# BloodAxe/pytorch-toolbelt

Measured on AMD Instinct MI355X. Metric: megapixels/sec tiled+d4-TTA merge on 5000x5000, higher is better.
Workload: dtype f32

## Files before the change

### pytorch_toolbelt_amd/csrc/ptb_bandplan.hip

```cpp
#include <algorithm>
#include <vector>

#include "ptb_view_device.h"

namespace ptb {

constexpr int PLAN_TILES = 224;
constexpr int PLAN_CH = 32;

struct BandItem {
    int ax, ay;
    int cwch;
    int ntiles;
    int partial;
    int pad[3];
    unsigned long long cover[MAX_COVER];
};
static_assert(sizeof(BandItem) == 64, "BandItem layout");

struct GroupTiles {
    const void* src[PLAN_TILES];
    long long vs[PLAN_TILES];
};

template <int NV, int CODES, int OPK, int LD, int CH = PLAN_CH, bool PF = false>
__global__ __launch_bounds__(16 * CH) void band_plan_kernel(const ViewArgs a, const BandItem* __restrict__ items, const GroupTiles t) {
    constexpr bool DB = PF && CH == 64 && lds_tiles(NV, CODES) > 0;
    constexpr int LDS_SET = lds_tiles(NV, CODES) * CW * CH;
    __shared__ __attribute__((aligned(16))) float lds[LDS_SET ? LDS_SET * (DB ? 2 : 1) : 4];
    const int tid = threadIdx.x;
    unsigned bid = blockIdx.x;
    if (a.ncells == 1) {
        const unsigned per_xcd = ((unsigned)a.total_chunks + 7u) / 8u;
        bid = (blockIdx.x & 7u) * per_xcd + (blockIdx.x >> 3);
        if (bid >= (unsigned)a.total_chunks) return;
    }
    int c = bid % a.C;
    unsigned item = bid / a.C;
    if (a.chan_loop) { c = 0; item = bid; }
    else if (a.ncells == 2) {
        const unsigned n_items = (unsigned)a.total_chunks / (unsigned)a.C;
        c = bid / n_items;
        item = bid - c * n_items;
    }
    const BandItem* __restrict__ it = items + item;
    const int cwch = it->cwch, partial = it->partial;
    const int cw = cwch & 0xffff, ch = cwch >> 16;
    const int q = tid & 15, r = tid >> 4;
    const bool act = (r < ch) && (4 * q < cw);
    const long long pix = (long long)(it->ay + r) * a.dst_row_stride + it->ax + 4 * q;
    float4 nfull = make_float4(1.f, 1.f, 1.f, 1.f);
    if (act && !partial) nfull = *reinterpret_cast<const float4*>(a.norm_full + pix);
    float4 acc = make_float4(0.f, 0.f, 0.f, 0.f);
    const int nt = it->ntiles;
    const bool rot = PF && a.rot_views && (item & 1u);
    constexpr bool ALL = PF && lds_tiles(NV, CODES) == 0 && NV <= 2 && CODES >= 0;
    if constexpr (ALL) {
        const int c_end = a.chan_loop ? a.C : c + 1;
        if (a.chan_loop) { c = 0; }
        float4 wv[MAX_COVER];
#pragma unroll
        for (int e = 0; e < MAX_COVER; ++e) {
            wv[e] = make_float4(0.f, 0.f, 0.f, 0.f);
            if (e < nt && act) {
                const unsigned long long cv = it->cover[e];
                const int lx = (int)((cv >> 16) & 0xffff), ly = (int)((cv >> 32) & 0xffff);
                wv[e] = *reinterpret_cast<const float4*>(a.weight + (long long)(ly + r) * a.W + lx + 4 * q);
            }
        }
        typename RawOf<LD>::type all[MAX_COVER][NV];
        auto request = [&](int cc) {
#pragma unroll
            for (int e = 0; e < MAX_COVER; ++e) {
                if (e < nt) {
                    const unsigned long long cv = it->cover[e];
                    const int slot = (int)(cv & 0xffff), lx = (int)((cv >> 16) & 0xffff), ly = (int)((cv >> 32) & 0xffff);
                    gather_load_raw<CH, NV, CODES, LD>(static_cast<const float*>(t.src[slot]), (long long)cc * a.H * a.W, t.vs[slot], a.nviews, a.codes, a.H,
                                                       a.W, lx, ly, cw, ch, tid, all[e]);
                }
            }
        };
        request(c);
        for (; c < c_end; ++c) {
            acc = make_float4(0.f, 0.f, 0.f, 0.f);
#pragma unroll
            for (int e = 0; e < MAX_COVER; ++e) {
                if (e < nt) {
                    float4 v[NV];
                    gather_widen<CH, NV, CODES, LD>(all[e], a.nviews, a.codes, cw, ch, tid, v);
                    float4 val = gather_tail<CH, NV, CODES, OPK>(v, a.nviews, a.codes, cw, ch, a.op, a.divisor, lds, tid, false);
                    val = round_src4<LD>(val, a.round_src);
                    acc.x = __fadd_rn(acc.x, __fmul_rn(val.x, wv[e].x));
                    acc.y = __fadd_rn(acc.y, __fmul_rn(val.y, wv[e].y));
                    acc.z = __fadd_rn(acc.z, __fmul_rn(val.z, wv[e].z));
                    acc.w = __fadd_rn(acc.w, __fmul_rn(val.w, wv[e].w));
                }
            }
            if (c + 1 < c_end) request(c + 1);
            if (act) {
                float* o = a.merged + (long long)c * a.dst_chan_stride + pix;
                if (partial) *reinterpret_cast<float4*>(o) = acc;
                else out_store4(o, make_float4(__fdiv_rn(acc.x, nfull.x), __fdiv_rn(acc.y, nfull.y), __fdiv_rn(acc.z, nfull.z), __fdiv_rn(acc.w, nfull.w)));
            }
        }
        return;
    }
    typename RawOf<LD>::type nxt[PF ? NV : 1];
    float4 wnxt = make_float4(0.f, 0.f, 0.f, 0.f);
    if constexpr (PF) {
        if (nt > 0) {
            const unsigned long long cv = it->cover[0];
            const int slot = (int)(cv & 0xffff), lx = (int)((cv >> 16) & 0xffff), ly = (int)((cv >> 32) & 0xffff);
            if (act) wnxt = *reinterpret_cast<const float4*>(a.weight + (long long)(ly + r) * a.W + lx + 4 * q);
            if (NV >= 2 && rot)
                gather_load_raw<CH, NV, CODES, LD, NV / 2>(static_cast<const float*>(t.src[slot]), (long long)c * a.H * a.W, t.vs[slot], a.nviews, a.codes, a.H,
                                                           a.W, lx, ly, cw, ch, tid, nxt);
            else
                gather_load_raw<CH, NV, CODES, LD>(static_cast<const float*>(t.src[slot]), (long long)c * a.H * a.W, t.vs[slot], a.nviews, a.codes, a.H, a.W, lx,
                                                   ly, cw, ch, tid, nxt);
        }
    }
    for (int e = 0; e < nt; ++e) {
        const unsigned long long cv = it->cover[e];
        const int slot = (int)(cv & 0xffff), lx = (int)((cv >> 16) & 0xffff), ly = (int)((cv >> 32) & 0xffff);
        float4 val;
        float4 w4 = make_float4(0.f, 0.f, 0.f, 0.f);
        if constexpr (PF) {
            float4 v[NV];
            gather_widen<CH, NV, CODES, LD>(nxt, a.nviews, a.codes, cw, ch, tid, v);
            w4 = wnxt;
            if (e + 1 < nt) {
                const unsigned long long cn = it->cover[e + 1];
                const int sn = (int)(cn & 0xffff), nlx = (int)((cn >> 16) & 0xffff), nly = (int)((cn >> 32) & 0xffff);
                if (act) wnxt = *reinterpret_cast<const float4*>(a.weight + (long long)(nly + r) * a.W + nlx + 4 * q);
                if (NV >= 2 && rot)
                    gather_load_raw<CH, NV, CODES, LD, NV / 2>(static_cast<const float*>(t.src[sn]), (long long)c * a.H * a.W, t.vs[sn], a.nviews, a.codes, a.H,
                                                               a.W, nlx, nly, cw, ch, tid, nxt);
                else
                    gather_load_raw<CH, NV, CODES, LD>(static_cast<const float*>(t.src[sn]), (long long)c * a.H * a.W, t.vs[sn], a.nviews, a.codes, a.H, a.W,
                                                       nlx, nly, cw, ch, tid, nxt);
            }
            const bool db = DB && a.lds_db;
            val = gather_tail<CH, NV, CODES, OPK>(v, a.nviews, a.codes, cw, ch, a.op, a.divisor, db ? lds + (e & 1) * LDS_SET : lds, tid, db ? false : e + 1 < nt);
        } else {
            val = gather_reduce<CH, NV, CODES, OPK, LD>(static_cast<const float*>(t.src[slot]), (long long)c * a.H * a.W, t.vs[slot],
                                                        a.nviews, a.codes, a.H, a.W, lx, ly, cw, ch, a.op, a.divisor, lds, tid,
                                                        e + 1 < nt);
            if (act) w4 = *reinterpret_cast<const float4*>(a.weight + (long long)(ly + r) * a.W + lx + 4 * q);
        }
        val = round_src4<LD>(val, a.round_src);
        if (act) {
            acc.x = __fadd_rn(acc.x, __fmul_rn(val.x, w4.x));
            acc.y = __fadd_rn(acc.y, __fmul_rn(val.y, w4.y));
            acc.z = __fadd_rn(acc.z, __fmul_rn(val.z, w4.z));
            acc.w = __fadd_rn(acc.w, __fmul_rn(val.w, w4.w));
        }
    }
    if (act) {
        float* o = a.merged + (long long)c * a.dst_chan_stride + pix;
        if (partial) *reinterpret_cast<float4*>(o) = acc;
        else out_store4(o, make_float4(__fdiv_rn(acc.x, nfull.x), __fdiv_rn(acc.y, nfull.y), __fdiv_rn(acc.z, nfull.z),
                                       __fdiv_rn(acc.w, nfull.w)));
    }
}

static void launch_plan(const ViewArgs& a, const BandItem* items, const GroupTiles& t, int blocks, int ch, hipStream_t s) {
    const dim3 grid(blocks), block(16 * ch);
    const bool nonlinear = a.op >= PTB_RED_GMEAN;
#define PTB_PLAN_PF(NV, CODES, LD)                                                                                  \
    do {                                                                                                            \
        if (ch == 64) {                                                                                             \
            if (nonlinear) hipLaunchKernelGGL((band_plan_kernel<NV, CODES, 1, LD, 64, true>), grid, block, 0, s, a, items, t); \
            else hipLaunchKernelGGL((band_plan_kernel<NV, CODES, 0, LD, 64, true>), grid, block, 0, s, a, items, t);       \
        } else if (nonlinear) hipLaunchKernelGGL((band_plan_kernel<NV, CODES, 1, LD, PLAN_CH, true>), grid, block, 0, s, a, items, t);    \
        else hipLaunchKernelGGL((band_plan_kernel<NV, CODES, 0, LD, PLAN_CH, true>), grid, block, 0, s, a, items, t);              \
    } while (0)
#define PTB_PLAN_LD(NV, CODES, LD)                                                                                  \
    do {                                                                                                            \
        if (ch == 64) {                                                                                             \
            if (nonlinear) hipLaunchKernelGGL((band_plan_kernel<NV, CODES, 1, LD, 64>), grid, block, 0, s, a, items, t); \
            else hipLaunchKernelGGL((band_plan_kernel<NV, CODES, 0, LD, 64>), grid, block, 0, s, a, items, t);       \
        } else if (nonlinear) hipLaunchKernelGGL((band_plan_kernel<NV, CODES, 1, LD>), grid, block, 0, s, a, items, t);    \
        else hipLaunchKernelGGL((band_plan_kernel<NV, CODES, 0, LD>), grid, block, 0, s, a, items, t);              \
    } while (0)
#define PTB_PLAN(NV, CODES)                                                                                         \
    do {                                                                                                            \
        if (a.in_dtype == PTB_F16) { if (g_band_half_pf) PTB_PLAN_PF(NV, CODES, 2); else PTB_PLAN_LD(NV, CODES, 2); }      \
        else if (a.in_dtype == PTB_BF16) { if (g_band_half_pf) PTB_PLAN_PF(NV, CODES, 3); else PTB_PLAN_LD(NV, CODES, 3); } \
        else if (g_band_half_pf >= 2) PTB_PLAN_PF(NV, CODES, 1);                                                    \
        else PTB_PLAN_LD(NV, CODES, 1);                                                                             \
    } while (0)
#define PTB_PLAN_RT(NV, CODES)           \
    do {                                                                                                            \
        if (a.in_dtype == PTB_F16) PTB_PLAN_LD(NV, CODES, 2);                                                       \
        else if (a.in_dtype == PTB_BF16) PTB_PLAN_LD(NV, CODES, 3);                                                 \
        else PTB_PLAN_LD(NV, CODES, 1);                                                                             \
    } while (0)
    if (a.nviews == 1 && a.codes == CODES_ID) PTB_PLAN(1, CODES_ID);
    else if (a.nviews == 2 && a.codes == CODES_FLIPLR) PTB_PLAN(2, CODES_FLIPLR);
    else if (a.nviews == 2 && a.codes == CODES_FLIPUD) PTB_PLAN(2, CODES_FLIPUD);
    else if (a.nviews == 3 && a.codes == CODES_FLIPS) PTB_PLAN(3, CODES_FLIPS);
    else if (a.nviews == 4 && a.codes == CODES_D2) PTB_PLAN(4, CODES_D2);
    else if (a.nviews == 8 && a.codes == CODES_D4) PTB_PLAN(8, CODES_D4);
    else PTB_PLAN_RT(8, -1);
#undef PTB_PLAN
#undef PTB_PLAN_RT
#undef PTB_PLAN_LD
#undef PTB_PLAN_PF
}

struct Group {
    int y0, y1;
    std::vector<int> tiles;
    int last_tile;
    long long item_off;
    int item_cnt;
};

}

struct ptb_band_plan {
    int n, C, th, tw, H, W;
    int ch = ptb::PLAN_CH;
    std::vector<int> xs, ys;
    std::vector<ptb::BandItem> items;
    std::vector<ptb::Group> groups;
    std::vector<int> last_group;
    std::vector<std::vector<int>> ready;
    std::vector<int> band_y0, band_y1, band_group;
    std::vector<char> group_launched;
    const ptb::BandItem* dev_items = nullptr;
    int n_bands = 0;
    int pos = 0, launched = 0;
    std::vector<const void*> src;
    std::vector<long long> vs;
    int cfg_set = 0, cfg_dtype = 0, cfg_V = 0, cfg_codes = 0, cfg_red = 0;
    int cfg_views[ptb::MAX_VIEWS] = {0};
    const void *cfg_merged = nullptr, *cfg_norm = nullptr, *cfg_weight = nullptr;
    struct Held { uintptr_t p0, p1; int last_group; };
    std::vector<Held> held;
    bool monotone = true;
};

using namespace ptb;

static int band_items(const ptb_band_plan& p, const std::vector<int>& cover, const std::vector<int>& slot_of, int y0, int y1, int partial,
                      std::vector<BandItem>& out) {
    std::vector<int> xe{0, p.W};
    for (int t : cover) { xe.push_back(p.xs[t]); xe.push_back(p.xs[t] + p.tw); }
    std::sort(xe.begin(), xe.end());
    xe.erase(std::unique(xe.begin(), xe.end()), xe.end());
    struct XCell { int ox, w, n; int tile[MAX_COVER]; };
    std::vector<XCell> cells;
    for (size_t xi = 0; xi + 1 < xe.size(); ++xi) {
        XCell c{};
        c.ox = xe[xi]; c.w = xe[xi + 1] - xe[xi];
        for (int t : cover) {
            if (p.xs[t] <= c.ox && c.ox < p.xs[t] + p.tw) {
                if (c.n == MAX_COVER) return PTB_EUNSUPPORTED;
                c.tile[c.n++] = t;
            }
        }
        if (!cells.empty() && cells.back().ox + cells.back().w == c.ox && cells.back().n == c.n &&
            std::equal(c.tile, c.tile + c.n, cells.back().tile)) {
            cells.back().w += c.w;
            continue;
        }
        cells.push_back(c);
    }
    for (const XCell& c : cells) {
        for (int cy = y0; cy < y1; cy += p.ch) {
            for (int cx = 0; cx < c.w; cx += CW) {
                BandItem it{};
                it.ax = c.ox + cx; it.ay = cy;
                it.cwch = std::min(CW, c.w - cx) | (std::min(p.ch, y1 - cy) << 16);
                it.ntiles = c.n;
                it.partial = partial;
                for (int e = 0; e < c.n; ++e) {
                    const int t = c.tile[e];
                    it.cover[e] = (unsigned long long)slot_of[t] | ((unsigned long long)(it.ax - p.xs[t]) << 16) |
                                  ((unsigned long long)(it.ay - p.ys[t]) << 32);
                }
                out.push_back(it);
            }
        }
    }
    return PTB_OK;
}

extern "C" int64_t ptb_band_plan_create(const int64_t* xs64, const int64_t* ys64, int n, int C, int th, int tw, int H, int W,
                                        int rows_per_launch, int final_lo, int final_hi, const int64_t* cuts, int ncuts,
                                        ptb_band_plan** out) {
    return ptb_band_plan_create2(xs64, ys64, n, C, th, tw, H, W, rows_per_launch, final_lo, final_hi, cuts, ncuts, nullptr, 0, out);
}

extern "C" int64_t ptb_band_plan_create2(const int64_t* xs64, const int64_t* ys64, int n, int C, int th, int tw, int H, int W,
                                         int rows_per_launch, int final_lo, int final_hi, const int64_t* cuts, int ncuts,
                                         const int64_t* early, int n_early, ptb_band_plan** out) {
    return ptb_band_plan_create3(xs64, ys64, n, C, th, tw, H, W, rows_per_launch, final_lo, final_hi, cuts, ncuts, early, n_early, 0, out);
}

extern "C" int64_t ptb_band_plan_create3(const int64_t* xs64, const int64_t* ys64, int n, int C, int th, int tw, int H, int W,
                                         int rows_per_launch, int final_lo, int final_hi, const int64_t* cuts, int ncuts,
                                         const int64_t* early, int n_early, int flags, ptb_band_plan** out) {
    const bool clip = (flags & 1) != 0;
    if (flags & ~1) return PTB_EINVAL;
    if (!xs64 || !ys64 || !out || n < 1 || C < 1 || th < 1 || tw < 1 || H < 1 || W < 1 || ncuts < 0 || (ncuts && !cuts)) return PTB_EINVAL;
    if (n_early < 0 || (n_early && !early)) return PTB_EINVAL;
    *out = nullptr;
    if (g_force_scalar || tw % 4 || th % 4 || W % 4 || tw > 32767 || th > 32767) return PTB_EUNSUPPORTED;
    ptb_band_plan* p = new ptb_band_plan();
    p->n = n; p->C = C; p->th = th; p->tw = tw; p->H = H; p->W = W;
    p->ch = g_band_rows;
    p->xs.resize(n); p->ys.resize(n);
    std::vector<int> edges{0, H};
    for (int t = 0; t < n; ++t) {
        if (xs64[t] < 0 || xs64[t] + tw > W) { delete p; return PTB_EBOUNDS; }
        if (!clip && (ys64[t] < 0 || ys64[t] + th > H)) { delete p; return PTB_EBOUNDS; }
        if (ys64[t] < -(int64_t)0x3fffffff || ys64[t] > (int64_t)0x3fffffff) { delete p; return PTB_EBOUNDS; }
        if (xs64[t] % 4 || ys64[t] % 4) { delete p; return PTB_EUNSUPPORTED; }
        p->xs[t] = (int)xs64[t]; p->ys[t] = (int)ys64[t];
        edges.push_back(std::min(std::max(p->ys[t], 0), H)); edges.push_back(std::min(std::max(p->ys[t] + th, 0), H));
    }
    std::vector<int> breaks;
    for (int k = 0; k < ncuts; ++k) {
        if (cuts[k] % 4) { delete p; return PTB_EUNSUPPORTED; }
        if (cuts[k] > 0 && cuts[k] < H) { edges.push_back((int)cuts[k]); breaks.push_back((int)cuts[k]); }
    }
    std::sort(edges.begin(), edges.end());
    edges.erase(std::unique(edges.begin(), edges.end()), edges.end());
    struct Band { int y0, y1; std::vector<int> cover; };
    std::vector<Band> bands;
    for (size_t i = 0; i + 1 < edges.size(); ++i) {
        Band b{edges[i], edges[i + 1], {}};
        for (int t = 0; t < n; ++t)
            if (p->ys[t] <= b.y0 && p->ys[t] + th >= b.y1) b.cover.push_back(t);
        if ((int)b.cover.size() > PLAN_TILES) { delete p; return PTB_EUNSUPPORTED; }
        bands.push_back(std::move(b));
    }
    p->n_bands = (int)bands.size();
    const int target = std::max(1, rows_per_launch);
    p->last_group.assign(n, -1);
    p->ready.assign(n, {});
    p->band_y0.resize(bands.size()); p->band_y1.resize(bands.size()); p->band_group.assign(bands.size(), -1);
    for (size_t b = 0; b < bands.size(); ++b) { p->band_y0[b] = bands[b].y0; p->band_y1[b] = bands[b].y1; }
    auto emit_group = [&](const std::vector<size_t>& members, const std::vector<int>& tiles) -> int {
// ... 129 lines not shown
    if (launched) *launched = p->launched;
    return PTB_OK;
}

extern "C" void ptb_band_plan_destroy(ptb_band_plan* p) { delete p; }

extern "C" int ptb_band_plan_submit(ptb_band_plan* p, int pos, int B, const void* batch, int64_t tile_stride, int64_t view_stride,
                                    int in_dtype, int V, const int* views, int reduction, float* merged, const float* norm_full,
                                    const float* weight, ptb_stream_t stream) {
    if (!p || !batch || !merged || !norm_full || !weight || B < 1) return PTB_EINVAL;
    if (!p->dev_items) return PTB_EINVAL;
    const int dtype_arg = in_dtype;
    in_dtype &= ~PTB_ROUND_SRC;
    if (reduction < PTB_RED_SUM || reduction > PTB_RED_LOG1P || in_dtype < PTB_F32 || in_dtype > PTB_BF16) return PTB_EINVAL;
    if (V < 1 || V > MAX_VIEWS || !views) return PTB_EINVAL;
    int nT = 0;
    for (int k = 0; k < V; ++k) {
        if (views[k] < 0 || views[k] > 7) return PTB_EINVAL;
        nT += views[k] & 1;
    }
    if (nT && p->th != p->tw) return PTB_EINVAL;
    if (pos != p->pos || pos + B > p->n) return PTB_EUNSUPPORTED;
    const int codes = [&] { int v = 0; for (int k = 0; k < V; ++k) v |= (views[k] & 7) << (3 * k); return v; }();
    if (p->cfg_set) {
        if (p->cfg_dtype != dtype_arg || p->cfg_V != V || p->cfg_codes != codes || p->cfg_red != reduction || p->cfg_merged != merged ||
            p->cfg_norm != norm_full || p->cfg_weight != weight) return PTB_EUNSUPPORTED;
    }
    const long long per_tile = (long long)p->C * p->th * p->tw;
    const unsigned mask = in_dtype == PTB_F32 ? 15u : 7u;
    const size_t esz = in_dtype == PTB_F32 ? 4 : 2;
    if (nT > MAX_T || tile_stride < per_tile || view_stride < per_tile || tile_stride % 4 || view_stride % 4 ||
        (reinterpret_cast<uintptr_t>(batch) & mask) || !aligned16(merged) || !aligned16(norm_full) || !aligned16(weight))
        return PTB_EUNSUPPORTED;
    p->cfg_set = 1; p->cfg_dtype = dtype_arg; p->cfg_V = V; p->cfg_codes = codes; p->cfg_red = reduction;
    for (int k = 0; k < V; ++k) p->cfg_views[k] = views[k];
    p->cfg_merged = merged; p->cfg_norm = norm_full; p->cfg_weight = weight;
    {
        int lg = 0;
        for (int b = 0; b < B; ++b) lg = std::max(lg, p->last_group[pos + b]);
        const uintptr_t p0 = reinterpret_cast<uintptr_t>(batch);
        p->held.push_back({p0, p0 + (size_t)((long long)(V - 1) * view_stride + (long long)(B - 1) * tile_stride + per_tile) * esz, lg});
    }
    for (int b = 0; b < B; ++b) {
        p->src[pos + b] = static_cast<const char*>(batch) + (size_t)b * (size_t)tile_stride * esz;
        p->vs[pos + b] = view_stride;
    }
    p->pos = pos + B;
    ViewArgs a{};
    a.weight = weight; a.merged = merged; a.norm_full = norm_full;
    a.in_dtype = in_dtype;
    a.round_src = (dtype_arg & PTB_ROUND_SRC) ? 1 : 0;
    a.rot_views = g_band_rot_views;
    a.lds_db = g_band_lds_db;
    a.H = p->th; a.W = p->tw; a.C = p->C;
    a.dst_chan_stride = (long long)p->H * p->W;
    a.dst_row_stride = p->W;
    a.nviews = V;
    a.codes = codes;
    a.scale = 1.0f;
    a.op = reduction;
    a.divisor = reduction == PTB_RED_SUM ? 1.0f : (float)V;
    int launched = 0;
    for (int t = pos; t < pos + B; ++t) {
        for (int gi : p->ready[t]) {
            const Group& g = p->groups[gi];
            p->group_launched[gi] = 1;
            if (!g.item_cnt) { ++p->launched; continue; }
            GroupTiles gt;
            for (size_t s = 0; s < g.tiles.size(); ++s) { gt.src[s] = p->src[g.tiles[s]]; gt.vs[s] = p->vs[g.tiles[s]]; }
            for (size_t s = g.tiles.size(); s < (size_t)PLAN_TILES; ++s) { gt.src[s] = nullptr; gt.vs[s] = 0; }
            a.chan_loop = (V == 1 && codes == CODES_ID && g_band_chan_loop && (in_dtype != PTB_F32 ? g_band_half_pf >= 1 : g_band_half_pf >= 2)) ? 1 : 0;
            const long long blocks = (long long)g.item_cnt * (a.chan_loop ? 1 : p->C);
            if (blocks > 0x7fffffffLL) return PTB_EUNSUPPORTED;
            a.ncells = a.chan_loop ? 0 : g_band_xcd; a.total_chunks = (int)blocks;
            launch_plan(a, p->dev_items + g.item_off, gt, a.ncells == 1 ? (int)(8 * ((blocks + 7) / 8)) : (int)blocks, p->ch, (hipStream_t)stream);
            const int rc = check_launch();
            if (rc != PTB_OK) return rc;
            ++p->launched;
            ++launched;
        }
    }
    if (launched || p->launched == (int)p->groups.size()) {
        if (p->launched == (int)p->groups.size()) p->held.clear();
        else if (p->monotone) {
            size_t k = 0;
            while (k < p->held.size() && p->held[k].last_group < p->launched) ++k;
            p->held.erase(p->held.begin(), p->held.begin() + (long)k);
        }
    }
    return launched;
}

extern "C" int ptb_band_plan_submit_next(ptb_band_plan* p, const void* batch, int B, ptb_stream_t stream) {
    if (!p || !batch || B < 1) return PTB_EINVAL;
    if (!p->cfg_set || p->pos + B > p->n) return PTB_EUNSUPPORTED;
    const int dt = p->cfg_dtype & ~PTB_ROUND_SRC;
    const size_t esz = dt == PTB_F32 ? 4 : 2;
    const long long per_tile = (long long)p->C * p->th * p->tw;
    const uintptr_t p0 = reinterpret_cast<uintptr_t>(batch), p1 = p0 + (size_t)((long long)p->cfg_V * B * per_tile) * esz;
    for (const ptb_band_plan::Held& h : p->held)
        if (h.p0 < p1 && p0 < h.p1) return PTB_EHELD;
    return ptb_band_plan_submit(p, p->pos, B, batch, per_tile, (long long)B * per_tile, p->cfg_dtype, p->cfg_V, p->cfg_views, p->cfg_red,
                                static_cast<float*>(const_cast<void*>(p->cfg_merged)), static_cast<const float*>(p->cfg_norm),
                                static_cast<const float*>(p->cfg_weight), stream);
}

extern "C" int ptb_band_plan_rows_launched(const ptb_band_plan* p, int r0, int r1) {
    if (!p || r1 < r0) return PTB_EINVAL;
    for (size_t b = 0; b < p->band_y0.size(); ++b)
        if (p->band_y0[b] < r1 && p->band_y1[b] > r0 && !p->group_launched[p->band_group[b]]) return 0;
    return 1;
}

template <int V>
__global__ __launch_bounds__(256) void halo_pack_kernel(const float* __restrict__ src, float* __restrict__ dst, int C, int rows, int cols,
                                                        long long cs, long long rs) {
    const long long per_row = cols / V;
    const long long total = (long long)C * rows * per_row;
    for (long long i = (long long)blockIdx.x * blockDim.x + threadIdx.x; i < total; i += (long long)gridDim.x * blockDim.x) {
        const long long x = i % per_row, cr = i / per_row;
        const long long r = cr % rows, c = cr / rows;
        const float* s = src + c * cs + r * rs + x * V;
        float* d = dst + i * V;
        if (V == 4) *reinterpret_cast<float4*>(d) = *reinterpret_cast<const float4*>(s);
        else d[0] = s[0];
    }
}

extern "C" int ptb_halo_pack(const float* src, int64_t chan_stride, int64_t row_stride, int C, int rows, int cols, float* dst,
                             ptb_stream_t stream) {
    if (!src || !dst || C < 1 || rows < 0 || cols < 0 || row_stride < cols || chan_stride < (int64_t)rows * row_stride) return PTB_EINVAL;
    if (rows == 0 || cols == 0) return PTB_OK;
    const bool vec = !g_force_scalar && cols % 4 == 0 && chan_stride % 4 == 0 && row_stride % 4 == 0 && aligned16(src) && aligned16(dst);
    const long long total = (long long)C * rows * (vec ? cols / 4 : cols);
    const int grid = (int)std::min<long long>((total + 255) / 256, 256 * 16);
    if (vec) hipLaunchKernelGGL(halo_pack_kernel<4>, dim3(grid), dim3(256), 0, (hipStream_t)stream, src, dst, C, rows, cols, (long long)chan_stride, (long long)row_stride);
    else hipLaunchKernelGGL(halo_pack_kernel<1>, dim3(grid), dim3(256), 0, (hipStream_t)stream, src, dst, C, rows, cols, (long long)chan_stride, (long long)row_stride);
    return check_launch();
}

extern "C" int ptb_band_plan_submit_rank(ptb_band_plan* p, int pos, int B, const void* batch, int64_t tile_stride, int64_t view_stride,
                                         int in_dtype, int V, const int* views, int reduction, float* merged, const float* norm_full,
                                         const float* weight, int n_sends, const int64_t* rects, float* const* send_bufs, int* packed,
                                         void* ready_event, int* all_packed, ptb_stream_t stream) {
    if (n_sends < 0 || (n_sends && (!rects || !send_bufs || !packed || !ready_event))) return PTB_EINVAL;
    const int rc = ptb_band_plan_submit(p, pos, B, batch, tile_stride, view_stride, in_dtype, V, views, reduction, merged, norm_full, weight, stream);
    if (rc < 0) return rc;
    int done = 0, fresh = 0;
    for (int k = 0; k < n_sends; ++k) {
        if (!packed[k] && rc > 0) {
            const int r0 = (int)rects[4 * k], r1 = (int)rects[4 * k + 1], c0 = (int)rects[4 * k + 2], c1 = (int)rects[4 * k + 3];
            if (r0 < 0 || r1 > p->H || c0 < 0 || c1 > p->W || r1 < r0 || c1 < c0 || !send_bufs[k]) return PTB_EINVAL;
            if (ptb_band_plan_rows_launched(p, r0, r1) == 1) {
                const int prc = ptb_halo_pack(merged + (long long)r0 * p->W + c0, (int64_t)p->H * p->W, p->W, p->C, r1 - r0, c1 - c0, send_bufs[k], stream);
                if (prc != PTB_OK) return prc;
                packed[k] = 1;
                ++fresh;
            }
        }
        done += packed[k] ? 1 : 0;
    }
    const bool all = done == n_sends;
    if (all && fresh && ready_event) {
        const hipError_t e = hipEventRecord((hipEvent_t)ready_event, (hipStream_t)stream);
        if (e != hipSuccess) { set_hip_error(e); return PTB_ELAUNCH; }
    }
    if (all_packed) *all_packed = all ? 1 : 0;
    return rc;
}

int ptb::g_band_chan_loop = 1;
int ptb::g_band_lds_db = 1;
int ptb::g_band_rot_views = 0;
int ptb::g_band_half_pf = 2;
int ptb::g_rank_finish_fused = 1;

struct FinishArgs {
    float* merged;
    const float* norm;
    int C, W;
    long long plane;
    int n_recvs, n_ranges;
    int r0[4], r1[4], c0[4], c1[4];
    const float* buf[4];
    int q0[2], q1[2];
};

__global__ __launch_bounds__(256) void band_finish_kernel(const FinishArgs a) {
    typedef float v4f __attribute__((ext_vector_type(4)));
    const int w4 = a.W >> 2;
    const int rows0 = a.q1[0] - a.q0[0];
    const long long total = (long long)(rows0 + (a.n_ranges > 1 ? a.q1[1] - a.q0[1] : 0)) * w4;
    for (long long i = (long long)blockIdx.x * blockDim.x + threadIdx.x; i < total; i += (long long)gridDim.x * blockDim.x) {
        const int t = (int)(i / w4), x = (int)(i - (long long)t * w4) * 4;
        const int r = t < rows0 ? a.q0[0] + t : a.q0[1] + (t - rows0);
        const v4f n = *reinterpret_cast<const v4f*>(a.norm + (long long)r * a.W + x);
        for (int c = 0; c < a.C; ++c) {
            float* mp = a.merged + c * a.plane + (long long)r * a.W + x;
            v4f v = *reinterpret_cast<const v4f*>(mp);
#pragma unroll
            for (int k = 0; k < 4; ++k) {
                if (k < a.n_recvs && r >= a.r0[k] && r < a.r1[k] && x >= a.c0[k] && x < a.c1[k]) {
                    const int cols = a.c1[k] - a.c0[k];
                    const v4f e = __builtin_nontemporal_load(reinterpret_cast<const v4f*>(
                        a.buf[k] + ((long long)c * (a.r1[k] - a.r0[k]) + (r - a.r0[k])) * cols + (x - a.c0[k])));
                    v.x = __fadd_rn(v.x, e.x); v.y = __fadd_rn(v.y, e.y); v.z = __fadd_rn(v.z, e.z); v.w = __fadd_rn(v.w, e.w);
                }
            }
            v4f o;
            o.x = __fdiv_rn(v.x, n.x); o.y = __fdiv_rn(v.y, n.y); o.z = __fdiv_rn(v.z, n.z); o.w = __fdiv_rn(v.w, n.w);
            __builtin_nontemporal_store(o, reinterpret_cast<v4f*>(mp));
        }
    }
}

extern "C" int ptb_band_plan_finish_rank(const ptb_band_plan* p, float* merged, const float* norm, int n_recvs, const int64_t* rects,
                                         const float* const* recv_bufs, int n_ranges, const int64_t* ranges, ptb_stream_t stream) {
    if (!p || !merged || !norm || n_recvs < 0 || n_ranges < 0 || (n_recvs && (!rects || !recv_bufs)) || (n_ranges && !ranges)) return PTB_EINVAL;
    const int64_t plane = (int64_t)p->H * p->W;
    for (int k = 0; k < n_recvs; ++k) {
        const int64_t r0 = rects[4 * k], r1 = rects[4 * k + 1], c0 = rects[4 * k + 2], c1 = rects[4 * k + 3];
        if (r0 < 0 || r1 > p->H || c0 < 0 || c1 > p->W || r1 < r0 || c1 < c0 || !recv_bufs[k]) return PTB_EINVAL;
    }
    for (int k = 0; k < n_ranges; ++k)
// ... 39 lines not shown
```

### pytorch_toolbelt_amd/csrc/ptb_common.h

```cpp
#pragma once
#include <hip/hip_runtime.h>
#include <stdint.h>

#include "../../include/ptb_hip.h"

namespace ptb {

void set_hip_error(hipError_t e);
void set_error_text(const char* text);

inline int check_launch() {
    hipError_t e = hipGetLastError();
    if (e != hipSuccess) {
        set_hip_error(e);
        return PTB_ELAUNCH;
    }
    return PTB_OK;
}

#ifndef PTB_NT_OUT
#define PTB_NT_OUT 1
#endif
__device__ __forceinline__ void out_store4(float* p, const float4 v) {
#if PTB_NT_OUT
    typedef float ptb_v4f __attribute__((ext_vector_type(4)));
    __builtin_nontemporal_store(ptb_v4f{v.x, v.y, v.z, v.w}, reinterpret_cast<ptb_v4f*>(p));
#else
    *reinterpret_cast<float4*>(p) = v;
#endif
}

__device__ __forceinline__ int wave_id() { return __builtin_amdgcn_readfirstlane((int)(threadIdx.x >> 6)); }

inline bool aligned16(const void* p) { return (reinterpret_cast<uintptr_t>(p) & 15u) == 0; }

extern int g_chunk_rows;
extern int g_force_scalar;
extern int g_loss_grid_cap;
extern int g_ms_tiled;
extern int g_ms_tile_w;
extern int g_rank_finish_fused;
extern int g_rs_xcd_map;
extern int g_lovasz_rankdot;
extern int g_lovasz_fused_dot;
extern int g_nt_grad_stores;
extern int g_stats_pk;
extern int g_focal_pk_grid;
extern int g_focal_pk;
extern int g_fused_pix2;
extern int g_loss_prefetch;
extern int g_smf_bwd_stash;
extern int g_band_rows;
extern int g_band_half_pf;
extern int g_band_chan_loop;
extern int g_band_lds_db;
extern int g_band_rot_views;
extern int g_band_xcd;
extern int g_ms_strip;
extern int g_ms_tile_rows;
extern int g_nt_loads;

}
```

### pytorch_toolbelt_amd/csrc/ptb_core.hip

```cpp
#include <algorithm>
#include <string>

#include "ptb_common.h"

namespace ptb {

static thread_local std::string g_last_error;
int g_chunk_rows = 32;
int g_force_scalar = 0;
int g_nt_loads = 1;
int g_band_xcd = 0;
int g_band_rows = 64;
int g_ms_tiled = 1;

void set_hip_error(hipError_t e) { g_last_error = hipGetErrorString(e); }
void set_error_text(const char* text) { g_last_error = text ? text : ""; }

template <bool NT>
__global__ __launch_bounds__(256) void merge_div_kernel(const float* __restrict__ image, const float* __restrict__ norm,
                                                        float* __restrict__ out, int C, long long hw4, long long ics4,
                                                        long long ocs4, const float* __restrict__ extra, long long ecs4,
                                                        long long en4) {
    typedef float v4f __attribute__((ext_vector_type(4)));
    const long long stride = (long long)gridDim.x * blockDim.x;
// ... 167 lines not shown
    }
    if (key == 3) {
        g_ms_tiled = value ? 1 : 0;
        return PTB_OK;
    }
    if (key == 4) {
        if (value < 0) return PTB_EINVAL;
        g_loss_grid_cap = value;
        return PTB_OK;
    }
    if (key == 5) {
        g_fused_pix2 = value ? 1 : 0;
        return PTB_OK;
    }
    if (key == 12) {
        if (value < 0 || value > 2) return PTB_EINVAL;
        g_focal_pk = value;
        return PTB_OK;
    }
    if (key == 15) {
        if (value != 64 && value != 128) return PTB_EINVAL;
        g_ms_tile_w = value;
        return PTB_OK;
    }
    if (key == 16) {
        g_nt_grad_stores = value ? 1 : 0;
        return PTB_OK;
    }
    if (key == 17) {
        g_rs_xcd_map = value & 7;
        return PTB_OK;
    }
    if (key == 18) {
        g_rank_finish_fused = value ? 1 : 0;
        return PTB_OK;
    }
    if (key == 19) {
        g_lovasz_fused_dot = value ? 1 : 0;
        return PTB_OK;
    }
    if (key == 20) {
        g_stats_pk = value ? 1 : 0;
        return PTB_OK;
    }
    if (key == 21) {
        g_band_half_pf = value < 0 ? 0 : (value > 2 ? 2 : value);
        return PTB_OK;
    }
    if (key == 22) {
        g_band_rot_views = value ? 1 : 0;
        return PTB_OK;
    }
    if (key == 27) {
        g_band_chan_loop = value ? 1 : 0;
        return PTB_OK;
    }
    if (key == 25) {
        g_band_lds_db = value ? 1 : 0;
        return PTB_OK;
    }
    if (key == 23) {
        g_lovasz_rankdot = value ? 1 : 0;
        return PTB_OK;
    }
    if (key == 13) {
        if (value < 1) return PTB_EINVAL;
        g_focal_pk_grid = value;
        return PTB_OK;
    }
    if (key == 6) {
        if (value != 16 && value != 32 && value != 64) return PTB_EINVAL;
        g_ms_tile_rows = value;
        return PTB_OK;
    }
    if (key == 11) {
        if (value != 32 && value != 64) return PTB_EINVAL;
        g_band_rows = value;
        return PTB_OK;
    }
    if (key == 10) {
        if (value < 0 || value > 2) return PTB_EINVAL;
        g_band_xcd = value;
        return PTB_OK;
    }
    if (key == 9) {
        if (value < 0 || value > 64) return PTB_EINVAL;
        g_ms_strip = value;
        return PTB_OK;
    }
    if (key == 8) {
        g_loss_prefetch = value ? 1 : 0;
        return PTB_OK;
    }
    if (key == 7) {
        if (value != 0 && value != 2 && value != 4) return PTB_EINVAL;
        g_smf_bwd_stash = value;
        return PTB_OK;
    }
    return PTB_EINVAL;
}

extern "C" int ptb_merge_div_ex(const float* image, const float* norm, float* out, int C, int64_t HW, int64_t image_cs,
                                int64_t out_cs, const float* extra, int64_t extra_cs, int64_t extra_n, ptb_stream_t stream) {
    if (!image || !norm || !out || C < 1 || HW < 0 || image_cs < HW || out_cs < HW) return PTB_EINVAL;
    if (extra_n < 0 || extra_n > HW || (extra_n > 0 && (!extra || extra_cs < extra_n))) return PTB_EINVAL;
    if (HW == 0) return PTB_OK;
    hipStream_t s = (hipStream_t)stream;
// ... 58 lines not shown
```

### pytorch_toolbelt_amd/csrc/ptb_view_device.h

```cpp
#pragma once
#include <initializer_list>

#include "ptb_common.h"

namespace ptb {

constexpr int MAX_VIEWS = 8;
constexpr int MAX_T = 4;
constexpr int MAX_CELLS = 64;
constexpr int MAX_COVER = 4;
constexpr int MAX_GROUP = 64;
constexpr int CW = 64;

constexpr int lds_tiles(int nv, int codes) {
    if (codes < 0) return nv < MAX_T ? nv : MAX_T;
    int n = 0;
    for (int k = 0; k < nv; ++k) n += (codes >> (3 * k)) & 1;
    return n;
}

struct Cell {
    int ox, oy, w, h;
    int chunk_end;
    int ntiles;
    int fresh;
    int final_;
    int tile[MAX_COVER];
};

struct CellArgs {
    Cell cells[MAX_CELLS];
    int tile_x[MAX_GROUP];
    int tile_y[MAX_GROUP];
    int tile_id[MAX_GROUP];
};

struct ViewArgs {
    const float* src;
    float* dst;
    float* norm;
    const float* weight;
    float* merged;
    const float* norm_full;
    int H, W, C;
    long long src_view_stride;
    long long src_tile_stride;
    long long dst_tile_stride;
    long long dst_chan_stride;
    int dst_row_stride;
    int nviews;
    int codes;
    int tiles_per_view;
    int src_tile_mod;
    int op;
    float divisor;
    float scale;
    int chunks_x, chunks_y;
    int ncells, total_chunks;
    int in_dtype;
    int keep_acc;
    int round_src;
    int chan_loop;
    int lds_db;
    int rot_views;
};

enum { MODE_REDUCE = 0, MODE_PERVIEW = 1, MODE_ACCUM = 2 };

constexpr float kEps = 1e-6f;
constexpr float kOneMinusEps = (float)(1.0 - 1e-6);

__device__ __forceinline__ float fast_exp(float x) { return __builtin_amdgcn_exp2f(x * 1.4426950408889634f); }
__device__ __forceinline__ float fast_log(float x) { return __builtin_amdgcn_logf(x) * 0.6931471805599453f; }
__device__ __forceinline__ float fast_rcp(float x) { return __builtin_amdgcn_rcpf(x); }

template <int OPK>
__device__ __forceinline__ float red_pre(float x, int op) {
    if (OPK == 0) return x;
    switch (op) {
        case PTB_RED_GMEAN: return fast_log(x);
        case PTB_RED_HMEAN: return fast_rcp(x < kEps ? kEps : x);
        case PTB_RED_HARMONIC1P: return fast_rcp(x + 1.0f);
        case PTB_RED_LOGODD: {
            float p = x < kEps ? kEps : (x > kOneMinusEps ? kOneMinusEps : x);
            return fast_log(p * fast_rcp(1.0f - p));
        }
        case PTB_RED_LOG1P: return fast_log(1.0f + x);
        default: return x;
    }
}

__device__ __forceinline__ float div_views(float s, float divisor) {
    const unsigned bits = __float_as_uint(divisor);
    if ((bits & 0x807FFFFFu) == 0 && bits != 0) return s * __uint_as_float(0x7F000000u - bits);
    return s / divisor;
}

template <int OPK>
__device__ __forceinline__ float red_post(float s, int op, float divisor) {
    if (OPK == 0) return divisor == 1.0f ? s : div_views(s, divisor);
    const float m = div_views(s, divisor);
    switch (op) {
        case PTB_RED_GMEAN: return fast_exp(m);
        case PTB_RED_HMEAN: return fast_rcp(m < kEps ? kEps : m);
        case PTB_RED_HARMONIC1P: return fast_rcp(m) - 1.0f;
        case PTB_RED_LOGODD: { const float e = fast_exp(m); return e * fast_rcp(1.0f + e); }
        case PTB_RED_LOG1P: return fast_exp(m) - 1.0f;
        default: return m;
    }
}

__device__ __forceinline__ float red_dpost(float out, int op) {
    switch (op) {
        case PTB_RED_GMEAN: return out;
        case PTB_RED_HMEAN: return out >= 1.0f / kEps ? 0.f : -out * out;
// ... 348 lines not shown
```

Before: 11590.

## Chunk channels per band workgroup and sum norm weights in-kernel

Replaces the all-or-one channel loop in the band plan kernel with a configurable channel chunk. The default walk picks the largest chunk that still leaves enough workgroups per CU, and the prefetch pipeline is flattened across tiles and channels so loads for the next channel overlap the current one. When the plan comes from the legacy create path, the normalisation divisor is summed from the weight tiles already loaded instead of read from a norm_full buffer, which saves that global read. It also adds XCD-grouped block ordering for chunked launches. The risks are lower occupancy, more register pressure from the flattened loop, and small rounding differences from computing the divisor in-kernel.

```diff
diff --git a/pytorch_toolbelt_amd/csrc/ptb_bandplan.hip b/pytorch_toolbelt_amd/csrc/ptb_bandplan.hip
--- a/pytorch_toolbelt_amd/csrc/ptb_bandplan.hip
+++ b/pytorch_toolbelt_amd/csrc/ptb_bandplan.hip
@@ -23,41 +23,50 @@
     long long vs[PLAN_TILES];
 };
 
+__device__ __forceinline__ long long band_pix(const ViewArgs& a, const BandItem* it, int r, int q) {
+    return (long long)(it->ay + r) * a.dst_row_stride + it->ax + 4 * q;
+}
+__device__ __forceinline__ void store_band(const ViewArgs& a, int c, long long pix, int partial, const float4 acc, const float4 nrm) {
+    float* o = a.merged + (long long)c * a.dst_chan_stride + pix;
+    if (partial) *reinterpret_cast<float4*>(o) = acc;
+    else out_store4(o, make_float4(__fdiv_rn(acc.x, nrm.x), __fdiv_rn(acc.y, nrm.y), __fdiv_rn(acc.z, nrm.z), __fdiv_rn(acc.w, nrm.w)));
+}
+
 template <int NV, int CODES, int OPK, int LD, int CH = PLAN_CH, bool PF = false>
 __global__ __launch_bounds__(16 * CH) void band_plan_kernel(const ViewArgs a, const BandItem* __restrict__ items, const GroupTiles t) {
     constexpr bool DB = PF && CH == 64 && lds_tiles(NV, CODES) > 0;
     constexpr int LDS_SET = lds_tiles(NV, CODES) * CW * CH;
     __shared__ __attribute__((aligned(16))) float lds[LDS_SET ? LDS_SET * (DB ? 2 : 1) : 4];
     const int tid = threadIdx.x;
-    unsigned bid = blockIdx.x;
+    const unsigned nck = (unsigned)a.n_chunks, n_items = (unsigned)a.total_chunks / nck;
+    unsigned bid = blockIdx.x, item, j;
     if (a.ncells == 1) {
         const unsigned per_xcd = ((unsigned)a.total_chunks + 7u) / 8u;
         bid = (blockIdx.x & 7u) * per_xcd + (blockIdx.x >> 3);
         if (bid >= (unsigned)a.total_chunks) return;
-    }
-    int c = bid % a.C;
-    unsigned item = bid / a.C;
-    if (a.chan_loop) { c = 0; item = bid; }
-    else if (a.ncells == 2) {
-        const unsigned n_items = (unsigned)a.total_chunks / (unsigned)a.C;
-        c = bid / n_items;
-        item = bid - c * n_items;
-    }
+        item = bid / nck; j = bid - item * nck;
+    } else if (a.ncells == 2) {
+        j = bid / n_items; item = bid - j * n_items;
+    } else if (a.chan_chunk > 1) {
+        const unsigned slot = bid >> 3, grp = slot / nck;
+        j = slot - grp * nck;
+        item = grp * 8u + (bid & 7u);
+        if (item >= n_items) return;
+    } else {
+        item = bid / nck; j = bid - item * nck;
+    }
+    const int c0 = (int)j * a.chan_chunk, c_end = min(a.C, c0 + a.chan_chunk);
     const BandItem* __restrict__ it = items + item;
     const int cwch = it->cwch, partial = it->partial;
     const int cw = cwch & 0xffff, ch = cwch >> 16;
     const int q = tid & 15, r = tid >> 4;
     const bool act = (r < ch) && (4 * q < cw);
-    const long long pix = (long long)(it->ay + r) * a.dst_row_stride + it->ax + 4 * q;
-    float4 nfull = make_float4(1.f, 1.f, 1.f, 1.f);
-    if (act && !partial) nfull = *reinterpret_cast<const float4*>(a.norm_full + pix);
-    float4 acc = make_float4(0.f, 0.f, 0.f, 0.f);
+    float4 nrm = make_float4(0.f, 0.f, 0.f, 0.f);
+    if (a.norm_load && act && !partial) nrm = *reinterpret_cast<const float4*>(a.norm_full + band_pix(a, it, r, q));
     const int nt = it->ntiles;
     const bool rot = PF && a.rot_views && (item & 1u);
     constexpr bool ALL = PF && lds_tiles(NV, CODES) == 0 && NV <= 2 && CODES >= 0;
     if constexpr (ALL) {
-        const int c_end = a.chan_loop ? a.C : c + 1;
-        if (a.chan_loop) { c = 0; }
         float4 wv[MAX_COVER];
 #pragma unroll
         for (int e = 0; e < MAX_COVER; ++e) {
@@ -66,6 +75,15 @@
                 const unsigned long long cv = it->cover[e];
                 const int lx = (int)((cv >> 16) & 0xffff), ly = (int)((cv >> 32) & 0xffff);
                 wv[e] = *reinterpret_cast<const float4*>(a.weight + (long long)(ly + r) * a.W + lx + 4 * q);
+            }
+        }
+        if (!a.norm_load) {
+#pragma unroll
+            for (int e = 0; e < MAX_COVER; ++e) {
+                if (e < nt) {
+                    nrm.x = __fadd_rn(nrm.x, wv[e].x); nrm.y = __fadd_rn(nrm.y, wv[e].y);
+                    nrm.z = __fadd_rn(nrm.z, wv[e].z); nrm.w = __fadd_rn(nrm.w, wv[e].w);
+                }
             }
         }
         typename RawOf<LD>::type all[MAX_COVER][NV];
@@ -80,9 +98,9 @@
                 }
             }
         };
-        request(c);
-        for (; c < c_end; ++c) {
-            acc = make_float4(0.f, 0.f, 0.f, 0.f);
+        request(c0);
+        for (int c = c0; c < c_end; ++c) {
+            float4 acc = make_float4(0.f, 0.f, 0.f, 0.f);
 #pragma unroll
             for (int e = 0; e < MAX_COVER; ++e) {
                 if (e < nt) {
@@ -97,11 +115,7 @@
                 }
             }
             if (c + 1 < c_end) request(c + 1);
-            if (act) {
-                float* o = a.merged + (long long)c * a.dst_chan_stride + pix;
-                if (partial) *reinterpret_cast<float4*>(o) = acc;
-                else out_store4(o, make_float4(__fdiv_rn(acc.x, nfull.x), __fdiv_rn(acc.y, nfull.y), __fdiv_rn(acc.z, nfull.z), __fdiv_rn(acc.w, nfull.w)));
-            }
+            if (act) store_band(a, c, band_pix(a, it, r, q), partial, acc, nrm);
         }
         return;
     }
@@ -113,39 +127,43 @@
             const int slot = (int)(cv & 0xffff), lx = (int)((cv >> 16) & 0xffff), ly = (int)((cv >> 32) & 0xffff);
             if (act) wnxt = *reinterpret_cast<const float4*>(a.weight + (long long)(ly + r) * a.W + lx + 4 * q);
             if (NV >= 2 && rot)
-                gather_load_raw<CH, NV, CODES, LD, NV / 2>(static_cast<const float*>(t.src[slot]), (long long)c * a.H * a.W, t.vs[slot], a.nviews, a.codes, a.H,
+                gather_load_raw<CH, NV, CODES, LD, NV / 2>(static_cast<const float*>(t.src[slot]), (long long)c0 * a.H * a.W, t.vs[slot], a.nviews, a.codes, a.H,
                                                            a.W, lx, ly, cw, ch, tid, nxt);
             else
-                gather_load_raw<CH, NV, CODES, LD>(static_cast<const float*>(t.src[slot]), (long long)c * a.H * a.W, t.vs[slot], a.nviews, a.codes, a.H, a.W, lx,
+                gather_load_raw<CH, NV, CODES, LD>(static_cast<const float*>(t.src[slot]), (long long)c0 * a.H * a.W, t.vs[slot], a.nviews, a.codes, a.H, a.W, lx,
                                                    ly, cw, ch, tid, nxt);
         }
     }
-    for (int e = 0; e < nt; ++e) {
+    const int nsteps = nt * (c_end - c0);
+    float4 acc = make_float4(0.f, 0.f, 0.f, 0.f);
+    int c = c0, e = 0;
+    for (int s = 0; s < nsteps; ++s) {
         const unsigned long long cv = it->cover[e];
         const int slot = (int)(cv & 0xffff), lx = (int)((cv >> 16) & 0xffff), ly = (int)((cv >> 32) & 0xffff);
+        const bool more = s + 1 < nsteps, last = e + 1 == nt;
         float4 val;
         float4 w4 = make_float4(0.f, 0.f, 0.f, 0.f);
         if constexpr (PF) {
             float4 v[NV];
             gather_widen<CH, NV, CODES, LD>(nxt, a.nviews, a.codes, cw, ch, tid, v);
             w4 = wnxt;
-            if (e + 1 < nt) {
-                const unsigned long long cn = it->cover[e + 1];
-                const int sn = (int)(cn & 0xffff), nlx = (int)((cn >> 16) & 0xffff), nly = (int)((cn >> 32) & 0xffff);
+            if (more) {
+                const int en = last ? 0 : e + 1, cn = last ? c + 1 : c;
+                const unsigned long long cvn = it->cover[en];
+                const int sn = (int)(cvn & 0xffff), nlx = (int)((cvn >> 16) & 0xffff), nly = (int)((cvn >> 32) & 0xffff);
                 if (act) wnxt = *reinterpret_cast<const float4*>(a.weight + (long long)(nly + r) * a.W + nlx + 4 * q);
                 if (NV >= 2 && rot)
-                    gather_load_raw<CH, NV, CODES, LD, NV / 2>(static_cast<const float*>(t.src[sn]), (long long)c * a.H * a.W, t.vs[sn], a.nviews, a.codes, a.H,
+                    gather_load_raw<CH, NV, CODES, LD, NV / 2>(static_cast<const float*>(t.src[sn]), (long long)cn * a.H * a.W, t.vs[sn], a.nviews, a.codes, a.H,
                                                                a.W, nlx, nly, cw, ch, tid, nxt);
                 else
-                    gather_load_raw<CH, NV, CODES, LD>(static_cast<const float*>(t.src[sn]), (long long)c * a.H * a.W, t.vs[sn], a.nviews, a.codes, a.H, a.W,
+                    gather_load_raw<CH, NV, CODES, LD>(static_cast<const float*>(t.src[sn]), (long long)cn * a.H * a.W, t.vs[sn], a.nviews, a.codes, a.H, a.W,
                                                        nlx, nly, cw, ch, tid, nxt);
             }
             const bool db = DB && a.lds_db;
-            val = gather_tail<CH, NV, CODES, OPK>(v, a.nviews, a.codes, cw, ch, a.op, a.divisor, db ? lds + (e & 1) * LDS_SET : lds, tid, db ? false : e + 1 < nt);
+            val = gather_tail<CH, NV, CODES, OPK>(v, a.nviews, a.codes, cw, ch, a.op, a.divisor, db ? lds + (s & 1) * LDS_SET : lds, tid, db ? false : more);
         } else {
             val = gather_reduce<CH, NV, CODES, OPK, LD>(static_cast<const float*>(t.src[slot]), (long long)c * a.H * a.W, t.vs[slot],
-                                                        a.nviews, a.codes, a.H, a.W, lx, ly, cw, ch, a.op, a.divisor, lds, tid,
-                                                        e + 1 < nt);
+                                                        a.nviews, a.codes, a.H, a.W, lx, ly, cw, ch, a.op, a.divisor, lds, tid, more);
             if (act) w4 = *reinterpret_cast<const float4*>(a.weight + (long long)(ly + r) * a.W + lx + 4 * q);
         }
         val = round_src4<LD>(val, a.round_src);
@@ -154,14 +172,21 @@
             acc.y = __fadd_rn(acc.y, __fmul_rn(val.y, w4.y));
             acc.z = __fadd_rn(acc.z, __fmul_rn(val.z, w4.z));
             acc.w = __fadd_rn(acc.w, __fmul_rn(val.w, w4.w));
-        }
-    }
-    if (act) {
-        float* o = a.merged + (long long)c * a.dst_chan_stride + pix;
-        if (partial) *reinterpret_cast<float4*>(o) = acc;
-        else out_store4(o, make_float4(__fdiv_rn(acc.x, nfull.x), __fdiv_rn(acc.y, nfull.y), __fdiv_rn(acc.z, nfull.z),
-                                       __fdiv_rn(acc.w, nfull.w)));
-    }
+            if (c == c0 && !a.norm_load) {
+                nrm.x = __fadd_rn(nrm.x, w4.x); nrm.y = __fadd_rn(nrm.y, w4.y);
+                nrm.z = __fadd_rn(nrm.z, w4.z); nrm.w = __fadd_rn(nrm.w, w4.w);
+            }
+        }
+        if (last) {
+            if (act) store_band(a, c, band_pix(a, it, r, q), partial, acc, nrm);
+            acc = make_float4(0.f, 0.f, 0.f, 0.f);
+            ++c; e = 0;
+        } else {
+            ++e;
+        }
+    }
+    if (nt == 0 && act)
+        for (c = c0; c < c_end; ++c) store_band(a, c, band_pix(a, it, r, q), partial, acc, nrm);
 }
 
 static void launch_plan(const ViewArgs& a, const BandItem* items, const GroupTiles& t, int blocks, int ch, hipStream_t s) {
@@ -209,6 +234,18 @@
 #undef PTB_PLAN_PF
 }
 
+constexpr int BAND_MIN_WG_PER_CU = 4;
+static int chan_chunk(int items, int C, int n_cu, bool walk) {
+    if (g_band_chan_chunk == 0) return 1;
+    if (g_band_chan_chunk >= 2) return std::min(g_band_chan_chunk, C);
+    if (!walk) return 1;
+    for (int n = 1; n < C; ++n) {
+        const int k = (C + n - 1) / n;
+        if ((long long)items * ((C + k - 1) / k) >= (long long)BAND_MIN_WG_PER_CU * n_cu) return k;
+    }
+    return 1;
+}
+
 struct Group {
     int y0, y1;
     std::vector<int> tiles;
@@ -231,6 +268,8 @@
     std::vector<char> group_launched;
     const ptb::BandItem* dev_items = nullptr;
     int n_bands = 0;
+    bool norm_in_kernel = false;
+    int n_cu = 0;
     int pos = 0, launched = 0;
     std::vector<const void*> src;
     std::vector<long long> vs;
@@ -291,7 +330,9 @@
 extern "C" int64_t ptb_band_plan_create(const int64_t* xs64, const int64_t* ys64, int n, int C, int th, int tw, int H, int W,
                                         int rows_per_launch, int final_lo, int final_hi, const int64_t* cuts, int ncuts,
                                         ptb_band_plan** out) {
-    return ptb_band_plan_create2(xs64, ys64, n, C, th, tw, H, W, rows_per_launch, final_lo, final_hi, cuts, ncuts, nullptr, 0, out);
+    const int64_t rc = ptb_band_plan_create2(xs64, ys64, n, C, th, tw, H, W, rows_per_launch, final_lo, final_hi, cuts, ncuts, nullptr, 0, out);
+    if (rc >= 0) (*out)->norm_in_kernel = true;
+    return rc;
 }
 
 extern "C" int64_t ptb_band_plan_create2(const int64_t* xs64, const int64_t* ys64, int n, int C, int th, int tw, int H, int W,
@@ -527,6 +568,15 @@
     a.round_src = (dtype_arg & PTB_ROUND_SRC) ? 1 : 0;
     a.rot_views = g_band_rot_views;
     a.lds_db = g_band_lds_db;
+    a.norm_load = (p->norm_in_kernel && g_band_norm_sum) ? 0 : 1;
+    a.ncells = g_band_xcd;
+    if (!p->n_cu) {
+        int dev = 0, n_cu = 0;
+        hipError_t e = hipGetDevice(&dev);
+        if (e == hipSuccess) e = hipDeviceGetAttribute(&n_cu, hipDeviceAttributeMultiprocessorCount, dev);
+        if (e != hipSuccess || n_cu < 1) { set_hip_error(e); return PTB_ELAUNCH; }
+        p->n_cu = n_cu;
+    }
     a.H = p->th; a.W = p->tw; a.C = p->C;
     a.dst_chan_stride = (long long)p->H * p->W;
     a.dst_row_stride = p->W;
@@ -535,6 +585,7 @@
     a.scale = 1.0f;
     a.op = reduction;
     a.divisor = reduction == PTB_RED_SUM ? 1.0f : (float)V;
+    const bool walk = V == 1 && codes == CODES_ID && (in_dtype != PTB_F32 ? g_band_half_pf >= 1 : g_band_half_pf >= 2);
     int launched = 0;
     for (int t = pos; t < pos + B; ++t) {
         for (int gi : p->ready[t]) {
@@ -544,11 +595,14 @@
             GroupTiles gt;
             for (size_t s = 0; s < g.tiles.size(); ++s) { gt.src[s] = p->src[g.tiles[s]]; gt.vs[s] = p->vs[g.tiles[s]]; }
             for (size_t s = g.tiles.size(); s < (size_t)PLAN_TILES; ++s) { gt.src[s] = nullptr; gt.vs[s] = 0; }
-            a.chan_loop = (V == 1 && codes == CODES_ID && g_band_chan_loop && (in_dtype != PTB_F32 ? g_band_half_pf >= 1 : g_band_half_pf >= 2)) ? 1 : 0;
-            const long long blocks = (long long)g.item_cnt * (a.chan_loop ? 1 : p->C);
+            a.chan_chunk = chan_chunk(g.item_cnt, p->C, p->n_cu, walk);
+            a.n_chunks = (p->C + a.chan_chunk - 1) / a.chan_chunk;
+            const long long total = (long long)g.item_cnt * a.n_chunks;
+            const long long blocks = a.ncells == 1 ? 8 * ((total + 7) / 8)
+                                   : (a.ncells == 0 && a.chan_chunk > 1 && a.n_chunks > 1) ? 8 * (((long long)g.item_cnt + 7) / 8) * a.n_chunks : total;
             if (blocks > 0x7fffffffLL) return PTB_EUNSUPPORTED;
-            a.ncells = a.chan_loop ? 0 : g_band_xcd; a.total_chunks = (int)blocks;
-            launch_plan(a, p->dev_items + g.item_off, gt, a.ncells == 1 ? (int)(8 * ((blocks + 7) / 8)) : (int)blocks, p->ch, (hipStream_t)stream);
+            a.total_chunks = (int)total;
+            launch_plan(a, p->dev_items + g.item_off, gt, (int)blocks, p->ch, (hipStream_t)stream);
             const int rc = check_launch();
             if (rc != PTB_OK) return rc;
             ++p->launched;
@@ -644,7 +698,8 @@
     return rc;
 }
 
-int ptb::g_band_chan_loop = 1;
+int ptb::g_band_chan_chunk = 1;
+int ptb::g_band_norm_sum = 1;
 int ptb::g_band_lds_db = 1;
 int ptb::g_band_rot_views = 0;
 int ptb::g_band_half_pf = 2;
diff --git a/pytorch_toolbelt_amd/csrc/ptb_common.h b/pytorch_toolbelt_amd/csrc/ptb_common.h
--- a/pytorch_toolbelt_amd/csrc/ptb_common.h
+++ b/pytorch_toolbelt_amd/csrc/ptb_common.h
@@ -52,7 +52,8 @@
 extern int g_smf_bwd_stash;
 extern int g_band_rows;
 extern int g_band_half_pf;
-extern int g_band_chan_loop;
+extern int g_band_chan_chunk;
+extern int g_band_norm_sum;
 extern int g_band_lds_db;
 extern int g_band_rot_views;
 extern int g_band_xcd;
diff --git a/pytorch_toolbelt_amd/csrc/ptb_core.hip b/pytorch_toolbelt_amd/csrc/ptb_core.hip
--- a/pytorch_toolbelt_amd/csrc/ptb_core.hip
+++ b/pytorch_toolbelt_amd/csrc/ptb_core.hip
@@ -243,7 +243,12 @@
         return PTB_OK;
     }
     if (key == 27) {
-        g_band_chan_loop = value ? 1 : 0;
+        if (value < 0) return PTB_EINVAL;
+        g_band_chan_chunk = value;
+        return PTB_OK;
+    }
+    if (key == 28) {
+        g_band_norm_sum = value ? 1 : 0;
         return PTB_OK;
     }
     if (key == 25) {
diff --git a/pytorch_toolbelt_amd/csrc/ptb_view_device.h b/pytorch_toolbelt_amd/csrc/ptb_view_device.h
--- a/pytorch_toolbelt_amd/csrc/ptb_view_device.h
+++ b/pytorch_toolbelt_amd/csrc/ptb_view_device.h
@@ -60,7 +60,9 @@
     int in_dtype;
     int keep_acc;
     int round_src;
-    int chan_loop;
+    int chan_chunk;
+    int n_chunks;
+    int norm_load;
     int lds_db;
     int rot_views;
 };
```

Result: faster. 11710, median of 6 (+1.1%).
